# gmarcais/Jellyfish

Hardware: AMD Instinct MI355X
Metric: k-mers/sec at k=21 canonical, 150 bp synthetic reads, bit-exact counts (higher is better)
Workload: dtype u64

## Files before the change

jellyfish_amd/csrc/kernels_p1ring.hip.hpp:

```cpp
#pragma once
#include <type_traits>
#include "kernels_part.hip.hpp"

namespace jfgpu {

template <int P> __device__ __forceinline__ void wave_prio() {
#if defined(__HIP_DEVICE_COMPILE__)
  __builtin_amdgcn_s_setprio(P);
#endif
}

__device__ __forceinline__ uint32_t adm_to_vmask(uint32_t adm) {
  uint32_t r = 0;
#pragma unroll
  for(int j = 0; j < 16; ++j) r |= ((adm >> j) & 1u) << (15 - j);
  return r;
}


constexpr uint32_t kStragPerBlock = 16384;

template <typename ITEM, uint32_t RB = 128> struct Ring {
  static constexpr uint32_t kSlots = RB / sizeof(ITEM);
  static constexpr uint32_t kUnit = 64 / sizeof(ITEM);
// ... 38 lines not shown
  const uint32_t w = s_fill[t];
  uint32_t cnt = w & 0xFFFFu; if(cnt > R::kSlots) cnt = R::kSlots;
  const uint32_t rb = (w >> 16) & (R::kSlots - 1);
  uint32_t units = cnt / R::kUnit; if(all && (cnt % R::kUnit)) ++units;
  uint32_t nout = 0;
  for(uint32_t s = 0; s < units; ++s) {
    uint4 v[4];
    const uint32_t s0 = (rb + s * R::kUnit) & (R::kSlots - 1);
#pragma unroll
    for(int q = 0; q < 4; ++q) v[q] = *reinterpret_cast<const uint4*>(s_ring + t * R::kSlots + ((s0 + R::kChunk * q) & (R::kSlots - 1)));
    if(!all) {
      uint32_t mx = 0;
#pragma unroll
      for(int q = 0; q < 4; ++q) { const uint32_t a = chunk_hole_key<ITEM>(v[q]); mx = mx > a ? mx : a; }
      if(mx == 0xFFFFFFFFu) break;
    }
    if constexpr(!OWNED) {
    if(B.room == 0 && B.nxt_asked) {
      if((uint64_t)B.nxt + kGran <= cap) { B.gpos = B.nxt; B.room = kGran; }
      else { B.exhausted = true; if(B.nxt < cap) atomicMax(&gshort[t], cap - B.nxt); }
      B.nxt_asked = false;
    }
    if(B.room == 0 && !B.exhausted) {
      const uint32_t r0 = atomicAdd(&gcur[t], kGran);
      if((uint64_t)r0 + kGran <= cap) { B.gpos = r0; B.room = kGran; }
      else { B.exhausted = true; if(r0 < cap) atomicMax(&gshort[t], cap - r0); }
    }
    }
    if(B.room) {
      uint4* dst = reinterpret_cast<uint4*>(my_region + B.gpos);
#pragma unroll
      for(int q = 0; q < 4; ++q) dst[q] = v[q];
      const uint32_t real = cnt - s * R::kUnit < R::kUnit ? cnt - s * R::kUnit : R::kUnit;
      B.gpos += OWNED ? real : R::kUnit; B.room -= R::kUnit; B.stored += real;
    } else {
#pragma unroll
      for(int q = 0; q < 4; ++q) chunk_items<ITEM>(v[q], [&](ITEM x) { if(x != hole) straggler(t, x, 1u); });
    }
#pragma unroll
    for(int q = 0; q < 4; ++q)
      *reinterpret_cast<uint4*>(s_ring + t * R::kSlots + ((s0 + R::kChunk * q) & (R::kSlots - 1))) = make_uint4(0xFFFFFFFFu, 0xFFFFFFFFu, 0xFFFFFFFFu, 0xFFFFFFFFu);
    ++nout;
  }
  if constexpr(!OWNED) { if(!all && !B.nxt_asked && !B.exhausted && B.room < R::kSlots) { B.nxt = atomicAdd(&gcur[t], kGran); B.nxt_asked = true; } }
  uint32_t expect = w;
  while(nout || (expect & 0xFFFFu) > R::kSlots) {
    uint32_t c = expect & 0xFFFFu; if(c > R::kSlots) c = R::kSlots;
    const uint32_t taken = nout * R::kUnit < c ? nout * R::kUnit : c;
    const uint32_t neww = ((((expect >> 16) + nout * R::kUnit) & 0xFFFFu) << 16) | (c - taken);
    const uint32_t old = atomicCAS(&s_fill[t], expect, neww);
    if(old == expect) break;
    expect = old;
  }
}

template <typename ITEM, uint32_t RB = 128>
__device__ __forceinline__ void ring_init(ITEM* s_ring, uint32_t* s_fill, uint32_t nb, uint32_t* s_nstrag) {
  using R = Ring<ITEM, RB>;
  for(uint32_t j = threadIdx.x; j < nb; j += blockDim.x) s_fill[j] = R::first_fill(j);
  uint4* r4 = reinterpret_cast<uint4*>(s_ring);
  for(uint32_t j = threadIdx.x; j < nb * (RB / 16) + RB / 16; j += blockDim.x) r4[j] = make_uint4(0xFFFFFFFFu, 0xFFFFFFFFu, 0xFFFFFFFFu, 0xFFFFFFFFu);
  if(threadIdx.x == 0) *s_nstrag = 0;
}

template <typename ITEM>
__device__ __forceinline__ void ring_finish(const RingBooks& B, uint32_t t, ITEM* my_region, uint32_t cap, unsigned int* gshort, unsigned long long* tot) {
  const ITEM hole = (ITEM)~(ITEM)0;
  for(uint32_t r = 0; r < B.room; ++r) my_region[B.gpos + r] = hole;
  if(B.nxt_asked) {
    if((uint64_t)B.nxt + kGran <= cap) { for(uint32_t r = 0; r < kGran; ++r) my_region[B.nxt + r] = hole; }
    else if(B.nxt < cap) atomicMax(&gshort[t], cap - B.nxt);
  }
  if(tot && B.stored) atomicAdd(&tot[t], (unsigned long long)B.stored);
}

struct OneWordDirect {
  static constexpr bool kCountsDirect = true;
  const DevTable* Tm; uint32_t b2; int returning;
  __device__ void operator()(uint32_t b, uint64_t item, uint32_t cnt) const { item_direct_call(Tm, b2, b, item, cnt, returning); }
};
struct RouteListDirect {
  static constexpr bool kCountsDirect = false;
  StragList SL;
  __device__ void operator()(uint32_t b, uint64_t item, uint32_t cnt) const {
    for(uint32_t i = 0; i < cnt; ++i) { const unsigned long long at = atomicAdd(SL.n, 1ull); if(at < SL.cap) SL.rec[at] = ((uint64_t)b << 32) | (uint32_t)item; }
  }
};

template <typename ITEM, bool BLOOM, int NB, int CANON, typename DIRECT = OneWordDirect>
__global__ __launch_bounds__(kPBlock) void p1_ring_kernel(DevTable T, DIRECT D, PartGeom P, const uint8_t* __restrict__ base,
                                                          int64_t lo, int64_t hi, uint32_t cap,
                                                          unsigned int* __restrict__ gcur,
                                                          unsigned long long* __restrict__ tot,
                                                          ITEM* __restrict__ out,
                                                          uint64_t* __restrict__ strag, uint32_t* __restrict__ strag_n) {
  using R = Ring<ITEM>;
  constexpr int RP = sizeof(ITEM) == 4 ? 8 : 4;
  JF_DYN_LDS(s_dyn);
  ITEM* s_ring = reinterpret_cast<ITEM*>(s_dyn);
  __shared__ uint64_t s_fwd[NB < 0 ? 1 : 8 * 256];
  __shared__ uint32_t s_fill[kGranMaxB + 32];
  __shared__ uint32_t s_nstrag;
  __shared__ uint32_t s_codes[kPBlock + 2];
  __shared__ uint32_t s_inv[kPBlock + 2];
  const TableGeom& g = T.g;
  const uint32_t nb = 1u << P.b1;
  const uint32_t t = threadIdx.x, lane = t & 63;
  const bool owner = t < nb;
  const ITEM hole = (ITEM)~(ITEM)0;
  if constexpr(NB >= 0) load_tables_lds(s_fwd, T.fwd_tbl, g.nbytes);
  ring_init<ITEM>(s_ring, s_fill, nb, &s_nstrag);
  const uint32_t dump = nb * R::kSlots + (lane & (R::kSlots - 1));
  [[maybe_unused]] const uint32_t xs_hi_mask = g.lsize_g > 32 ? (g.lsize_g >= 64 ? 0xFFFFFFFFu : ((1u << (g.lsize_g - 32)) - 1u)) : 0u;
  unsigned int* const gshort = gcur + nb;
  uint64_t* const my_strag = strag + (size_t)blockIdx.x * kStragPerBlock * R::kWords;
  const uint32_t k = g.k, bshift = g.lsize_l - P.b1;
  const uint32_t rc_shift = 2 * (k - 1);
  const uint32_t rest_mask = P.rest_shift >= 32 ? 0xFFFFFFFFu : ((1u << P.rest_shift) - 1u);
  RingBooks B;
  if(owner) { B.nxt = atomicAdd(&gcur[t], kGran); B.nxt_asked = true; }
  ITEM* const my_region = out + (uint64_t)t * cap;
  uint32_t my_mers = 0, my_direct = 0;

  auto straggler = [&](uint32_t b, ITEM item, uint32_t cnt) {
    const uint32_t at = atomicAdd(&s_nstrag, 1u);
    if(at < kStragPerBlock) strag_store<ITEM>(my_strag + (size_t)at * R::kWords, b, item, cnt);
    else { D(b, (uint64_t)item, cnt); ++my_direct; }
  };

  const int64_t n_tiles = (hi + kPTilePos - 1) / kPTilePos;
  TileRaw Rw = tile_fetch(base, (int64_t)blockIdx.x * kPTilePos, lo, hi);
  lds_barrier();
  [[maybe_unused]] PhaseClk pc;
  for(int64_t tile = blockIdx.x; tile < n_tiles; tile += gridDim.x) {
    const LaneWords L = tile_stage(Rw, tile * kPTilePos, lo, hi, s_codes, s_inv);
    Rw = tile_fetch(base, (tile + gridDim.x) * kPTilePos, lo, hi);
    JF_PHASE(pc, 0);
    const uint32_t adm = BLOOM ? bloom_admit_mask(T.bloom, g, L) : 0xFFFFu;
    uint64_t fw = (((uint64_t)L.p2 << 32) | L.p1) & g.key_mask;
    uint64_t rc = revcomp64(fw, k);
    uint64_t smear = L.inv48;
    for(uint32_t s = 1; s < k; ) { const uint32_t step = s < k - s ? s : k - s; smear |= smear >> step; s += step; }
    const uint32_t rawmask = ~(uint32_t)smear & 0xFFFFu;
    const uint32_t vmask = BLOOM ? (rawmask & adm_to_vmask(adm)) : rawmask;
    my_mers += (uint32_t)__popc(rawmask);
    auto rounds = [&](auto runs_tag) {
    constexpr bool RUNS = decltype(runs_tag)::value;
    uint64_t pk = 0; uint32_t pv = 0, run = 0;
#pragma unroll 1
    for(int j0 = 0; j0 < kPerLane; j0 += RP) {
      constexpr int NE = RUNS ? RP + 1 : RP;
      uint32_t ea[NE], eo[NE]; ITEM ei[NE];
      [[maybe_unused]] uint32_t spm = 0;
#pragma unroll
      for(int e = 0; e < NE; ++e) { ea[e] = dump; ei[e] = 0; eo[e] = 0; }
      auto emit = [&](int e, uint64_t key, uint32_t cnt, bool on) {
        uint32_t b; ITEM item;
        if constexpr(NB == kHashXS && sizeof(ITEM) == 4) {
          uint32_t ylo, yhi;
          xs_hash_halves<false>((uint32_t)key, (uint32_t)(key >> 32), xs_hi_mask, ylo, yhi);
          b = funnel_r(yhi, ylo, bshift) & (nb - 1);
          item = ((ylo & rest_mask) << g.rem_bits) | ((uint32_t)(key >> 32) >> (g.lsize_g - 32));
        } else {
          const uint64_t pos = NB < 0 ? xs_hash(key, g.lsize_g, g.key_bits) : hash_tables_t<(NB < 0 ? 0 : NB)>(s_fwd, key, g.nbytes);
          b = (uint32_t)(pos >> bshift) & (nb - 1);
          if constexpr(sizeof(ITEM) == 4) item = (((uint32_t)pos & rest_mask) << g.rem_bits) | (uint32_t)(key >> g.lsize_g);
          else item = make_item<ITEM>(g, P, key, pos & g.local_mask);
        }
        const bool special = on && (item == hole || cnt > 1);
        const bool normal = on && !special;
#ifndef JFGPU_P1_LATE_SPECIAL
        if(special) straggler(b, item, cnt);
        const uint32_t o = atomicAdd(&s_fill[normal ? b : nb + (lane & 31u)], 1u);
        ea[e] = normal ? b * R::kSlots : dump; ei[e] = item; eo[e] = normal ? o : 0u;
#else
        const uint32_t o = atomicAdd(&s_fill[normal ? b : nb + (lane & 31u)], 1u);
        spm |= special ? 1u << e : 0u;
        ea[e] = on ? b * R::kSlots : dump; ei[e] = item; eo[e] = normal ? o : special ? (R::kFull | ((cnt < 0xFFFFu ? cnt : 0xFFFFu) << 16)) : 0u;
#endif
      };
#ifndef JFGPU_P1_OLD_EXTRACT
      const uint32_t cur_r = L.cur << (2 * j0), ncur_r = ~cur_r, vm_r = vmask << j0;
#endif
#pragma unroll
      for(int e = 0; e < RP; ++e) {
#ifndef JFGPU_P1_OLD_EXTRACT
        const uint32_t c = (cur_r >> (2 * (15 - e))) & 3u, nc = (ncur_r >> (2 * (15 - e))) & 3u;
        const uint32_t v = vm_r & (1u << (15 - e));
#else
        const int j = j0 + e;
        const uint32_t c = (L.cur >> (2 * (15 - j))) & 3u, nc = 3u - c;
        const uint32_t v = vmask & (1u << (15 - j));
#endif
        if constexpr(NB >= 5 || NB == kHashXS) {
          const uint32_t flo = (uint32_t)fw, fhi = (uint32_t)(fw >> 32), rlo = (uint32_t)rc, rhi = (uint32_t)(rc >> 32);
          fw = ((uint64_t)(funnel_r(fhi, flo, 30) & (uint32_t)(g.key_mask >> 32)) << 32) | ((flo << 2) | c);
          rc = ((uint64_t)((rhi >> 2) | (nc << (rc_shift - 32))) << 32) | funnel_r(rhi, rlo, 2);
        } else {
          fw = ((fw << 2) | c) & g.key_mask;
          rc = (rc >> 2) | ((uint64_t)nc << rc_shift);
        }
        const uint64_t key = ((CANON == 1 || (CANON == 2 && g.canonical)) && rc < fw) ? rc : fw;
        if constexpr(RUNS) {
#ifdef JFGPU_P1_NO_RUNS
          const bool same = false;
#else
          const bool same = v && pv && key == pk;
#endif
          emit(e, pk, run, pv && !same);
          run = same ? run + 1 : 1;
          pk = key; pv = v;
        } else emit(e, key, 1u, v != 0);
      }
      if constexpr(RUNS) { if(j0 + RP >= kPerLane) { emit(NE - 1, pk, run, pv != 0); pv = 0; } }
      uint32_t ghosts = 0;
#pragma unroll
      for(int e = 0; e < NE; ++e) {
        const uint32_t full = eo[e] & R::kFull;
        ghosts |= full;
        const uint32_t at = ea[e] + ((eo[e] + (eo[e] >> 16)) & (R::kSlots - 1));
        s_ring[full ? dump : at] = ei[e];
      }
      if(ghosts) {
#pragma unroll 1
#ifndef JFGPU_P1_LATE_SPECIAL
        for(int e = 0; e < NE; ++e) {
          uint32_t a = 0, o = 0; ITEM it = 0;
#pragma unroll
          for(int q = 0; q < NE; ++q) if(q == e) { a = ea[q]; o = eo[q]; it = ei[q]; }
          if(o & R::kFull) straggler(a / R::kSlots, it, 1u);
        }
#else
        for(int e = 0; e < NE; ++e) if(eo[e] & R::kFull) straggler(ea[e] / R::kSlots, ei[e], ((spm >> e) & 1u) ? eo[e] >> 16 : 1u);
#endif
      }
      JF_PHASE(pc, 1);
      lds_barrier();
      JF_PHASE(pc, 2);
#ifndef JFGPU_P1_NO_FLUSH_PRIO
      wave_prio<3>();
#endif
      if(owner) ring_flush<ITEM>(s_ring, s_fill, t, false, B, my_region, cap, gcur, gshort, straggler);
#ifndef JFGPU_P1_NO_FLUSH_PRIO
      wave_prio<0>();
#endif
      JF_PHASE(pc, 3);
    }
    };
    bool may_run = k < 14;
    {
      const uint32_t hc = L.cur ^ (L.cur >> 2), hp = L.p1 ^ (L.p1 >> 2);
      may_run = may_run || (hc & 0x3FFFu) == 0 || ((hc >> 16) & 0x3FFFu) == 0 || (hp & 0x3FFFu) == 0;
    }
#ifdef JFGPU_P1_ALWAYS_RUNS
    may_run = true;
#endif
    if(__ballot(may_run) != 0ull) rounds(std::true_type{}); else rounds(std::false_type{});
  }
  lds_barrier();
  if(owner) { ring_flush<ITEM>(s_ring, s_fill, t, true, B, my_region, cap, gcur, gshort, straggler); ring_finish<ITEM>(B, t, my_region, cap, gshort, tot); }
  lds_barrier();
  if(t == 0) strag_n[blockIdx.x] = s_nstrag < kStragPerBlock ? s_nstrag : kStragPerBlock;
  JF_PHASE(pc, 4);
  JF_PHASE_FLUSH(pc, 0);
  if(DIRECT::kCountsDirect && my_direct) atomicAdd((unsigned long long*)&T.counters[CTR_DIRECT], (unsigned long long)my_direct);
  uint64_t w = my_mers;
  for(int o = 32; o > 0; o >>= 1) w += __shfl_down(w, o, 64);
  if((threadIdx.x & 63) == 0 && w) atomicAdd((unsigned long long*)&T.counters[CTR_MERS], (unsigned long long)w);
}

template <typename ITEM, typename DIRECT>
__global__ __launch_bounds__(256) void p1_stragglers_kernel(DIRECT D, unsigned long long* __restrict__ ctr_direct, const uint64_t* __restrict__ strag,
                                                            const uint32_t* __restrict__ strag_n, uint32_t n_lists, uint32_t cap,
                                                            unsigned int* __restrict__ gcur, unsigned long long* __restrict__ tot,
                                                            ITEM* __restrict__ out, uint32_t list_cap = kStragPerBlock) {
  using R = Ring<ITEM>;
  uint32_t my_direct = 0;
  for(uint32_t l = blockIdx.x; l < n_lists; l += gridDim.x) {
    const uint32_t n = strag_n[l];
    const uint64_t* rec = strag + (size_t)l * list_cap * R::kWords;
    for(uint32_t i = threadIdx.x; i < n; i += blockDim.x) {
      uint32_t b, cnt; ITEM item;
      strag_load<ITEM>(rec + (size_t)i * R::kWords, b, item, cnt);
      if(cnt == 1 && item != (ITEM)~(ITEM)0) {
        const uint32_t at = atomicAdd(&gcur[b], 1u);
        if(at < cap) { out[(uint64_t)b * cap + at] = item; if(tot) atomicAdd(&tot[b], 1ull); continue; }
        atomicMin(&gcur[b], cap);
// ... 115 lines not shown
        for(int e = 0; e < RP; ++e) it[e] = nx[e];
        r0 += RS;
        load_full(k + 1 < n_full ? r0 : my_a, nx);
        process(it);
      }
    }
    if(r0 < my_b) { uint32_t it[RP]; load_partial(r0, it); process(it); }
  }
  lds_barrier();
  flush(true);
  if(owner) ring_finish<uint32_t>(B, t, my_region, cap, gs, tot ? tot + dest0 : nullptr);
  lds_barrier();
  if(t == 0) strag_n[list] = s_nstrag < kP2StragPerBlock ? s_nstrag : kP2StragPerBlock;
  if(my_direct) atomicAdd(ctr_direct, (unsigned long long)my_direct);
}

template <typename ITEM, int NV, typename DIRECT, int PD = 1>
__global__ __launch_bounds__(kPBlock) void p2_ring_roles_kernel(DIRECT D, uint32_t b2e, uint32_t tag_bits, SegList S, uint32_t cap,
                                                                unsigned int* __restrict__ gcur, ITEM* __restrict__ out, uint32_t bucket0,
                                                                uint64_t* __restrict__ strag, uint32_t* __restrict__ strag_n, unsigned long long* __restrict__ ctr_direct) {
  using R = Ring<ITEM>;
  constexpr int VPI = (int)R::kChunk;
  constexpr int RP = NV * VPI;
  constexpr uint32_t kHalf = kPBlock / 2;
  constexpr uint64_t RS = (uint64_t)kHalf * RP;
  JF_DYN_LDS(s_dyn);
  ITEM* s_ring = reinterpret_cast<ITEM*>(s_dyn);
  __shared__ uint32_t s_fill[kGranMaxB];
  __shared__ uint32_t s_nstrag;
  const uint32_t nb = 1u << b2e;
  const uint32_t bucket = bucket0 + blockIdx.x;
  const uint32_t dest0 = bucket * nb;
  const uint32_t t = threadIdx.x, lane = t & 63;
  const bool storer = t < kHalf;
  const ITEM hole = (ITEM)~(ITEM)0;
  ring_init<ITEM>(s_ring, s_fill, nb, &s_nstrag);
  const uint32_t dump = nb * R::kSlots + (lane & (R::kSlots - 1));
  uint64_t* const my_strag = strag + (size_t)blockIdx.x * kP2StragPerBlock * R::kWords;
  uint32_t my_direct = 0;
  auto straggler = [&](uint32_t d, ITEM item, uint32_t cnt) {
    const uint32_t at = atomicAdd(&s_nstrag, 1u);
    if(at < kP2StragPerBlock) strag_store<ITEM>(my_strag + (size_t)at * R::kWords, dest0 + d, item, cnt);
    else { D(dest0 + d, item, cnt); ++my_direct; }
  };
  lds_barrier();
  auto seg_bounds = [&](uint32_t seg, uint64_t& a, uint64_t& b) { a = seg_lo(S, seg, bucket); b = seg_hi(S, seg, bucket); };
  if(storer) {
    const uint32_t d0 = t, d1 = t + kHalf;
    const bool has0 = d0 < nb, has1 = d1 < nb;
    RingBooks B0, B1;
    B0.room = B1.room = cap & ~(R::kUnit - 1);
    ITEM* const r0p = out + ((uint64_t)dest0 + d0) * cap;
    ITEM* const r1p = out + ((uint64_t)dest0 + d1) * cap;
    auto flush = [&](bool all) {
      if(has0) ring_flush<ITEM, true>(s_ring, s_fill, d0, all, B0, r0p, cap, gcur, gcur, straggler);
      if(has1) ring_flush<ITEM, true>(s_ring, s_fill, d1, all, B1, r1p, cap, gcur, gcur, straggler);
    };
    for(uint32_t seg = 0; seg < S.n; ++seg) {
      uint64_t a, b; seg_bounds(seg, a, b);
      const uint64_t rounds = (b - a + RS - 1) / RS;
#pragma unroll 1
      for(uint64_t r = 0; r < rounds; ++r) { lds_barrier(); flush(false); }
    }
    lds_barrier();
    flush(true);
    if(has0) gcur[dest0 + d0] = B0.gpos;
    if(has1) gcur[dest0 + d1] = B1.gpos;
  } else {
    const uint32_t l = t - kHalf;
    for(uint32_t seg = 0; seg < S.n; ++seg) {
      uint64_t a, b; seg_bounds(seg, a, b);
      const ITEM* src = reinterpret_cast<const ITEM*>(S.items[seg]);
      auto load_full = [&](uint64_t r0, ITEM (&it)[RP]) {
#pragma unroll
        for(int h = 0; h < NV; ++h) {
          const uint4 v = *reinterpret_cast<const uint4*>(src + r0 + (uint64_t)h * kHalf * VPI + (uint64_t)VPI * l);
          int q = 0;
          chunk_items<ITEM>(v, [&](ITEM x) { it[VPI * h + q] = x; ++q; });
        }
      };
      auto load_partial = [&](uint64_t r0, ITEM (&it)[RP]) {
#pragma unroll
        for(int h = 0; h < NV; ++h) {
          const uint64_t i = r0 + (uint64_t)h * kHalf * VPI + (uint64_t)VPI * l;
#pragma unroll
          for(int q = 0; q < VPI; ++q) it[VPI * h + q] = i + q < b ? src[i + q] : hole;
        }
      };
      auto load_exact = [&](uint64_t r0, ITEM (&it)[RP]) {
#pragma unroll 1
        for(int h = 0; h < NV; ++h) {
          const uint64_t i = r0 + (uint64_t)h * kHalf * VPI + (uint64_t)VPI * l;
#pragma unroll
          for(int q = 0; q < VPI; ++q) {
            ITEM x = hole;
            if(i + q < b) { x = src[i + q]; if(x == hole) straggler((uint32_t)(x >> tag_bits) & (nb - 1), x, 1u); }
            it[VPI * h + q] = x;
          }
        }
      };
      auto append = [&](const ITEM (&it)[RP]) {
        uint32_t ea[RP], eo[RP];
#pragma unroll
        for(int e = 0; e < RP; ++e) {
          ea[e] = dump; eo[e] = 0;
          if(it[e] != hole) { const uint32_t d = (uint32_t)(it[e] >> tag_bits) & (nb - 1); ea[e] = d * R::kSlots; eo[e] = atomicAdd(&s_fill[d], 1u); }
        }
        uint32_t ghosts = 0;
#pragma unroll
        for(int e = 0; e < RP; ++e) {
          const uint32_t full = eo[e] & R::kFull;
          ghosts |= full;
          const uint32_t at = ea[e] + ((eo[e] + (eo[e] >> 16)) & (R::kSlots - 1));
          s_ring[full ? dump : at] = it[e];
        }
        if(ghosts) {
#pragma unroll 1
          for(int e = 0; e < RP; ++e) if(eo[e] & R::kFull) straggler(ea[e] / R::kSlots, it[e], 1u);
        }
        lds_barrier();
      };
      uint64_t r0 = a;
      if(S.sh[seg] == 0) {
#pragma unroll 1
        for(; r0 < b; r0 += RS) { ITEM it[RP]; load_exact(r0, it); append(it); }
        continue;
      }
      const uint64_t n_full = (b - a) / RS;
      if(n_full) {
        ITEM nx[PD][RP];
#pragma unroll
        for(int d = 0; d < PD; ++d) load_full((uint64_t)d < n_full ? a + (uint64_t)d * RS : a, nx[d]);
        uint64_t k = 0;
#pragma unroll 1
        for(; k + PD <= n_full; k += PD) {
#pragma unroll
          for(int d = 0; d < PD; ++d) {
            ITEM it[RP];
#pragma unroll
            for(int e = 0; e < RP; ++e) it[e] = nx[d][e];
            const uint64_t nxt = k + d + PD;
            load_full(nxt < n_full ? a + nxt * RS : a, nx[d]);
            append(it);
          }
        }
#pragma unroll
        for(int d = 0; d < PD - 1; ++d)
          if(k + d < n_full) append(nx[d]);
        r0 = a + n_full * RS;
      }
      if(r0 < b) { ITEM it[RP]; load_partial(r0, it); append(it); }
    }
    lds_barrier();
  }
  lds_barrier();
  if(t == 0) strag_n[blockIdx.x] = s_nstrag < kP2StragPerBlock ? s_nstrag : kP2StragPerBlock;
  if(my_direct) atomicAdd(ctr_direct, (unsigned long long)my_direct);
}

}
```

jellyfish_amd/csrc/kmer_core.hpp:

```cpp
#pragma once
#include <stdint.h>

#if defined(__HIPCC__)
#define JF_HD __host__ __device__ __forceinline__
#else
#define JF_HD inline
#endif

namespace jfgpu {

constexpr uint32_t kMaxTileBits = 13;
constexpr uint32_t kMinCountBits = 16;
constexpr uint32_t kMinCountBits32 = 8;

JF_HD uint32_t base_code(uint32_t c) {
  const uint32_t u = c & 0xDFu;
  const uint32_t x = (u >> 1) & 3u;
  const uint32_t code = x ^ (x >> 1);
  const uint32_t valid_set = (1u << 1) | (1u << 3) | (1u << 7) | (1u << 20);
  const bool ok = ((u ^ 0x40u) < 32u) && ((valid_set >> (u & 31u)) & 1u);
  return ok ? code : 4u;
}

JF_HD uint32_t letters_of_codes(uint32_t code) {
// ... 246 lines not shown
JF_HD uint32_t probe_lin(uint32_t idx0, uint32_t p, uint32_t tile_mask) {
  return ((idx0 & ~((1u << kBucketBits) - 1u)) + p) & tile_mask;
}

JF_HD void load16(const uint8_t* p, uint32_t w[4]) {
#if defined(__HIP_DEVICE_COMPILE__)
  const uint4 v = *reinterpret_cast<const uint4*>(p);
  w[0] = v.x; w[1] = v.y; w[2] = v.z; w[3] = v.w;
#else
  for(int i = 0; i < 4; ++i)
    w[i] = (uint32_t)p[4 * i] | ((uint32_t)p[4 * i + 1] << 8) | ((uint32_t)p[4 * i + 2] << 16) | ((uint32_t)p[4 * i + 3] << 24);
#endif
}

constexpr int kPerLane = 16;

JF_HD void load_pack16(const uint8_t* __restrict__ base, int64_t off, int64_t lo, int64_t hi,
                                   uint32_t& codes, uint32_t& inval) {
  if(off + 16 <= lo || off >= hi || off < 0) { codes = 0; inval = 0xFFFFu; return; }
  uint32_t w[4];
  if(off + 16 <= hi) {
    load16(base + off, w);
  } else {
    w[0] = w[1] = w[2] = w[3] = 0;
    for(int i = 0; i < 16 && off + i < hi; ++i) w[i >> 2] |= (uint32_t)base[off + i] << (8 * (i & 3));
  }
  pack16(w, codes, inval);
  if(off < lo) inval |= (0xFFFFu << (16 - (int)(lo - off))) & 0xFFFFu;
  if(off + 16 > hi) inval |= (1u << (int)(off + 16 - hi)) - 1u;
}

struct LaneWords {
  uint32_t cur, p1, p2;
  uint64_t inv48;
};

template <typename F>
JF_HD void for_each_kmer(const TableGeom& g, const LaneWords& L, F&& f) {
  const uint32_t k = g.k;
  uint64_t fw = (((uint64_t)L.p2 << 32) | L.p1) & g.key_mask;
  uint64_t rc = revcomp64(fw, k);
  const uint64_t kwin = k >= 64 ? ~0ull : ((1ull << k) - 1);
  const uint32_t rc_shift = 2 * (k - 1);
#pragma unroll
  for(int j = 0; j < kPerLane; ++j) {
    const uint64_t c = (L.cur >> (2 * (15 - j))) & 3u;
    fw = ((fw << 2) | c) & g.key_mask;
    rc = (rc >> 2) | ((3ull - c) << rc_shift);
    const bool valid = ((L.inv48 >> (15 - j)) & kwin) == 0;
    if(valid) f(j, (g.canonical && rc < fw) ? rc : fw);
  }
}

}
```

jellyfish_amd/csrc/jfgpu.hip:

```cpp
#include <hip/hip_runtime.h>
#include <math.h>
#include <stdint.h>
#include <stdio.h>
#include <string.h>
#include <algorithm>
#include <array>
#include <chrono>
#include <memory>
#include <numeric>
#include <string>
#include <type_traits>
#include <vector>

#include "../../include/jfgpu.h"
#include "gf2_matrix.hpp"
#include "tuning.hpp"
#include "kernels.hip.hpp"
#include "kernels_part.hip.hpp"
#include "kernels_tile.hip.hpp"
#include "kernels_p1ring.hip.hpp"
#include "kernels_bloom.hip.hpp"
#include "kernels_bloom_part.hip.hpp"
#include "kernels_wide.hip.hpp"
#include "kernels_wide_part.hip.hpp"
// ... 676 lines not shown
}

void jfgpu_destroy(jfgpu_table* t) {
  if(!t) return;
  hipSetDevice(t->device);
  if(t->stream) hipStreamSynchronize(t->stream);
  prof_collect(t);
  part_discard(t);
  t->stream2.sync();
  delete t;
}

int jfgpu_get_info(const jfgpu_table* t, jfgpu_info* o) {
  if(!t || !o) return fail(JFGPU_E_INVALID, "null argument");
  memset(o, 0, sizeof(*o));
  o->k = t->g.k; o->key_len = t->g.key_bits; o->canonical = t->g.canonical;
  o->lsize = t->g.lsize_g; o->size = 1ull << t->g.lsize_g; o->local_size = 1ull << t->g.lsize_l;
  o->shard_bits = t->g.shard_bits; o->shard_id = t->g.shard_id;
  o->val_len = t->g.cnt_bits; o->slot_bytes = (uint32_t)slot_bytes_of(t); o->tile_slots = 1u << t->g.tile_bits;
  o->matrix_identity = t->matrix.identity ? 1 : 0;
  o->out_counter_len = t->out_counter_len;
  o->max_reprobe = t->dt.max_probe;
  o->table_bytes = (1ull << t->g.lsize_l) * slot_bytes_of(t);
  return JFGPU_OK;
}

int jfgpu_get_matrix(const jfgpu_table* t, uint64_t* columns) {
  if(!t || !columns) return fail(JFGPU_E_INVALID, "null argument");
  memcpy(columns, t->matrix.columns.data(), sizeof(uint64_t) * t->matrix.c);
  return JFGPU_OK;
}

int jfgpu_clear(jfgpu_table* t) {
  if(t) { t->failed = 0; t->failed_msg.clear(); }
  int rc = use(t); if(rc) return rc;
  part_discard(t);
  HIP_TRY(hipMemsetAsync(t->dt.slots, 0, (1ull << t->g.lsize_l) * slot_bytes_of(t), t->stream));
  HIP_TRY(hipMemsetAsync(t->dt.ovf_key, 0, t->ovf_cap * sizeof(uint64_t), t->stream));
  HIP_TRY(hipMemsetAsync(t->dt.ovf_cnt, 0, t->ovf_cap * sizeof(uint64_t), t->stream));
  HIP_TRY(hipMemsetAsync(t->dt.counters, 0, CTR_COUNT * sizeof(uint64_t), t->stream));
  HIP_TRY(hipMemsetAsync(t->dt.dirty, 0, (size_t)1 << (t->g.lsize_l - t->g.tile_bits), t->stream));
  HIP_TRY(hipStreamSynchronize(t->stream));
  t->pristine = true; t->occ_known = 0; t->fed_since = 0; t->direct_seen = 0; t->occ_bound = 0; t->bigval_bound = 0; t->ovf_failed_need = 0;
  t->flushes_plain = 0; t->flushes_heavy = 0;
  t->n_p2_roles = t->n_p2_ring = t->n_p2_sort = t->n_p2_exact = t->n_p1_ring = t->n_p1_other = t->n_tile_dense = t->n_tile_nword = 0;
  return JFGPU_OK;
}

int jfgpu_sync(jfgpu_table* t) {
  int rc = use(t); if(rc) return rc;
  rc = part_flush(t); if(rc) return rc;
  HIP_TRY(hipStreamSynchronize(t->stream));
#ifdef JFGPU_PHASE_PROF
  { unsigned long long c[24], z[24] = {0};
    if(hipMemcpyFromSymbol(c, HIP_SYMBOL(g_phase_prof), sizeof c) == hipSuccess) {
      fprintf(stderr, "[phase prof] P1 (ring): stage %llu  encode+hash+append %llu  (barrier) %llu  units out %llu  finish %llu\n",
              c[0], c[1], c[2], c[3], c[4]);
      fprintf(stderr, "[phase prof] P2: (barrier) %llu  load %llu  hist %llu  scan %llu  lds-scatter %llu  write-out %llu  finish %llu\n",
              c[8], c[9], c[10], c[11], c[12], c[13], c[14]);
      fprintf(stderr, "[phase prof] T: loop+offsets %llu  rank adds + fill %llu  place %llu  merge %llu  queue (wave 0's own) %llu  (its wait for the others) %llu  store %llu\n",
              c[16], c[17], c[18], c[22], c[21], c[19], c[20]);
      (void)hipMemcpyToSymbol(HIP_SYMBOL(g_phase_prof), z, sizeof z);
    } }
#endif
#ifdef JFGPU_TILE_PROF
  { uint64_t c[CTR_COUNT]; if(read_counters(t, c) == JFGPU_OK)
      fprintf(stderr, "[tile prof] wait+prefetch %llu  fill %llu  insert %llu  store %llu (shader clocks, summed over blocks)\n",
              (unsigned long long)c[CTR_PROF0], (unsigned long long)c[CTR_PROF0 + 1], (unsigned long long)c[CTR_PROF0 + 2], (unsigned long long)c[CTR_PROF0 + 3]); }
#endif
  return check_deferred(t);
}

int jfgpu_wait(jfgpu_table* t) {
  int rc = use(t); if(rc) return rc;
  HIP_TRY(hipStreamSynchronize(t->stream));
  return JFGPU_OK;
}

int jfgpu_count_ascii_dev(jfgpu_table* t, const char* d_bases, size_t n) {
  int rc = use(t); if(rc) return rc;
  if(t->g.shard_bits) return fail(JFGPU_E_INVALID, "sharded table: count through its communicator (jfgpu_comm_count_ascii_dev)");
  if(!d_bases && n) return fail(JFGPU_E_INVALID, "null buffer");
  return launch_count(t, d_bases, n);
}

int jfgpu_count_ascii(jfgpu_table* t, const char* bases, size_t n) {
  int rc = use(t); if(rc) return rc;
  if(t->g.shard_bits) return fail(JFGPU_E_INVALID, "sharded table: count through its communicator (jfgpu_comm_count_ascii_dev)");
  if(!bases && n) return fail(JFGPU_E_INVALID, "null buffer");
  if(n < t->g.k) return JFGPU_OK;
  rc = ensure_stage(t); if(rc) return rc;
  const size_t step = kStageBytes - (t->g.k - 1);
  for(size_t o = 0; o < n; o += step) {
    const size_t len = std::min(kStageBytes, n - o);
    const int b = t->stage_next; t->stage_next ^= 1;
    HIP_TRY(hipEventSynchronize(t->stage_done[b]));
    HIP_TRY(hipMemcpyAsync(t->d_stage[b], bases + o, len, hipMemcpyHostToDevice, t->stream));
    rc = launch_count(t, (const char*)t->d_stage[b].get(), len); if(rc) return rc;
    HIP_TRY(hipEventRecord(t->stage_done[b], t->stream));
    if(o + len >= n) break;
  }
  return JFGPU_OK;
}

static int add_keys_piece(jfgpu_table* t, const uint64_t* d_keys, size_t n, uint64_t val, uint8_t* d_is_new) {
  int rc = JFGPU_OK;
  if(!n) return JFGPU_OK;
  { const bool big = t->g.cnt_bits < 64 && (val >> t->g.cnt_bits) != 0;
    rc = ensure_ovf(t, big ? 0 : (uint64_t)n * val, big ? n : 0); if(rc) return rc; }
  const bool one_word = !t->wide && !t->nword;
  if(one_word && val == 1 && !d_is_new && use_partitioned(t, n * 8)) {
    const int prc = part_ingest(t, (const uint8_t*)d_keys, 0, (int64_t)n, true, n);
    if(prc >= 0) return prc;
  }
// ... 517 lines not shown
```

jellyfish_amd/csrc/kernels.hip.hpp:

```cpp
#pragma once
#include <hip/hip_runtime.h>
#include <stdint.h>
#include "kmer_core.hpp"

namespace jfgpu {

constexpr int kBlock = 256;
constexpr int kPerThread = kPerLane;
constexpr int kTilePos = kBlock * kPerThread;

enum Counter : int { CTR_FULL = 0, CTR_MERS = 1, CTR_OVF_FULL = 2, CTR_OVF_USED = 3, CTR_MISROUTED = 4, CTR_DIRECT = 5,
                     CTR_T_ITEMS = 6, CTR_T_QUEUED = 7 ,
                     CTR_PROF0 = 8 , CTR_COUNT = 12 };

#ifdef JFGPU_PHASE_PROF
__device__ unsigned long long g_phase_prof[24];
struct PhaseClk {
  long long acc[8] = {0, 0, 0, 0, 0, 0, 0, 0}; long long t;
  __device__ PhaseClk() { t = clock64(); }
  __device__ void mark(int i) { const long long n = clock64(); acc[i] += n - t; t = n; }
  __device__ void flush(int base) { if(threadIdx.x == 0) for(int i = 0; i < 8; ++i) if(acc[i]) atomicAdd(&g_phase_prof[base + i], (unsigned long long)acc[i]); }
};
#define JF_PHASE(pc, i) (pc).mark(i)
#define JF_PHASE_FLUSH(pc, base) (pc).flush(base)
#else
struct PhaseClk {};
#define JF_PHASE(pc, i) do {} while(0)
#define JF_PHASE_FLUSH(pc, base) do {} while(0)
#endif

struct DevBloom {
  uint32_t* data;
  uint64_t m;
  uint64_t recip;
  uint32_t nh;
  uint32_t nbytes;
  uint32_t kind;
  uint32_t pad_;
  const uint64_t* tbl1;
  const uint64_t* tbl2;
  uint64_t* cache;
  uint64_t cache_mask;
};

struct DevTable {
  TableGeom g;
  uint64_t* slots;
  const uint64_t* fwd_tbl;
  const uint64_t* inv_tbl;
  uint64_t* ovf_key;
  uint64_t* ovf_cnt;
  uint64_t ovf_mask;
  uint64_t* counters;
  uint32_t max_probe;
  DevBloom bloom;
  uint8_t* dirty;
};

#if defined(JFGPU_EMU)
__device__ __forceinline__ void lds_barrier() { __syncthreads(); }
#define JF_DYN_LDS(name) unsigned char* name = ::hip_emu::dyn_lds()
#else
__device__ __forceinline__ void lds_barrier() { asm volatile("s_waitcnt lgkmcnt(0)\n\ts_barrier" ::: "memory"); }
#define JF_DYN_LDS(name) extern __shared__ __align__(16) unsigned char name[]
#endif

__device__ inline bool bloom_admits(const DevBloom& B, uint64_t key);
__device__ inline uint32_t bloom_admit_mask(const DevBloom& B, const TableGeom& g, const LaneWords& L);

__device__ inline void ovf_add(const DevTable& T, uint64_t slot, uint64_t units) {
  const uint64_t want = slot + 1;
  uint64_t h = (slot * 0x9E3779B97F4A7C15ull) >> 20;
  for(uint64_t p = 0; p <= T.ovf_mask; ++p) {
    const uint64_t s = (h + p) & T.ovf_mask;
    unsigned long long old = atomicCAS((unsigned long long*)&T.ovf_key[s], 0ull, (unsigned long long)want);
    if(old == 0ull) atomicAdd((unsigned long long*)&T.counters[CTR_OVF_USED], 1ull);
    if(old == 0ull || old == want) {
      atomicAdd((unsigned long long*)&T.ovf_cnt[s], (unsigned long long)units);
      return;
    }
  }
// ... 908 lines not shown
```

Before: 15.78 billion.

## Extract k-mers by direct funnel shifts and use mask-select bitops in emit

```diff
diff --git a/jellyfish_amd/csrc/kernels_p1ring.hip.hpp b/jellyfish_amd/csrc/kernels_p1ring.hip.hpp
--- a/jellyfish_amd/csrc/kernels_p1ring.hip.hpp
+++ b/jellyfish_amd/csrc/kernels_p1ring.hip.hpp
@@ -177,7 +177,11 @@
   unsigned int* const gshort = gcur + nb;
   uint64_t* const my_strag = strag + (size_t)blockIdx.x * kStragPerBlock * R::kWords;
   const uint32_t k = g.k, bshift = g.lsize_l - P.b1;
-  const uint32_t rc_shift = 2 * (k - 1);
+  constexpr bool EXTRACT = NB >= 5 || NB == kHashXS;
+  constexpr bool MASKS = EXTRACT;
+  [[maybe_unused]] const uint32_t bo_mask = (nb - 1) << 2;
+  [[maybe_unused]] const uint32_t spare_bo = (nb + (lane & 31u)) << 2;
+  [[maybe_unused]] const uint32_t rc_shift = 2 * (k - 1), hi_bits = 2 * k - 32;
   const uint32_t rest_mask = P.rest_shift >= 32 ? 0xFFFFFFFFu : ((1u << P.rest_shift) - 1u);
   RingBooks B;
   if(owner) { B.nxt = atomicAdd(&gcur[t], kGran); B.nxt_asked = true; }
@@ -199,8 +203,10 @@
     Rw = tile_fetch(base, (tile + gridDim.x) * kPTilePos, lo, hi);
     JF_PHASE(pc, 0);
     const uint32_t adm = BLOOM ? bloom_admit_mask(T.bloom, g, L) : 0xFFFFu;
-    uint64_t fw = (((uint64_t)L.p2 << 32) | L.p1) & g.key_mask;
-    uint64_t rc = revcomp64(fw, k);
+    [[maybe_unused]] uint64_t fw = 0, rc = 0;
+    [[maybe_unused]] RcString V{};
+    if constexpr(EXTRACT) V = rc_string(L, k);
+    else { fw = (((uint64_t)L.p2 << 32) | L.p1) & g.key_mask; rc = revcomp64(fw, k); }
     uint64_t smear = L.inv48;
     for(uint32_t s = 1; s < k; ) { const uint32_t step = s < k - s ? s : k - s; smear |= smear >> step; s += step; }
     const uint32_t rawmask = ~(uint32_t)smear & 0xFFFFu;
@@ -212,53 +218,43 @@
 #pragma unroll 1
     for(int j0 = 0; j0 < kPerLane; j0 += RP) {
       constexpr int NE = RUNS ? RP + 1 : RP;
-      uint32_t ea[NE], eo[NE]; ITEM ei[NE];
-      [[maybe_unused]] uint32_t spm = 0;
-#pragma unroll
-      for(int e = 0; e < NE; ++e) { ea[e] = dump; ei[e] = 0; eo[e] = 0; }
-      auto emit = [&](int e, uint64_t key, uint32_t cnt, bool on) {
+      uint32_t ea[NE], eo[NE]; [[maybe_unused]] uint32_t em[NE]; ITEM ei[NE];
+#pragma unroll
+      for(int e = 0; e < NE; ++e) { ea[e] = MASKS ? 0u : dump; ei[e] = 0; eo[e] = 0; em[e] = 0; }
+      auto emit = [&](int e, uint64_t key, uint32_t cnt, uint32_t m) {
         uint32_t b; ITEM item;
         if constexpr(NB == kHashXS && sizeof(ITEM) == 4) {
           uint32_t ylo, yhi;
           xs_hash_halves<false>((uint32_t)key, (uint32_t)(key >> 32), xs_hi_mask, ylo, yhi);
-          b = funnel_r(yhi, ylo, bshift) & (nb - 1);
+          b = funnel_r(yhi, ylo, bshift - 2) & bo_mask;
           item = ((ylo & rest_mask) << g.rem_bits) | ((uint32_t)(key >> 32) >> (g.lsize_g - 32));
         } else {
           const uint64_t pos = NB < 0 ? xs_hash(key, g.lsize_g, g.key_bits) : hash_tables_t<(NB < 0 ? 0 : NB)>(s_fwd, key, g.nbytes);
-          b = (uint32_t)(pos >> bshift) & (nb - 1);
+          b = ((uint32_t)(pos >> bshift) & (nb - 1)) << (MASKS ? 2 : 0);
           if constexpr(sizeof(ITEM) == 4) item = (((uint32_t)pos & rest_mask) << g.rem_bits) | (uint32_t)(key >> g.lsize_g);
           else item = make_item<ITEM>(g, P, key, pos & g.local_mask);
         }
-        const bool special = on && (item == hole || cnt > 1);
-        const bool normal = on && !special;
-#ifndef JFGPU_P1_LATE_SPECIAL
-        if(special) straggler(b, item, cnt);
-        const uint32_t o = atomicAdd(&s_fill[normal ? b : nb + (lane & 31u)], 1u);
-        ea[e] = normal ? b * R::kSlots : dump; ei[e] = item; eo[e] = normal ? o : 0u;
-#else
-        const uint32_t o = atomicAdd(&s_fill[normal ? b : nb + (lane & 31u)], 1u);
-        spm |= special ? 1u << e : 0u;
-        ea[e] = on ? b * R::kSlots : dump; ei[e] = item; eo[e] = normal ? o : special ? (R::kFull | ((cnt < 0xFFFFu ? cnt : 0xFFFFu) << 16)) : 0u;
-#endif
+        if constexpr(MASKS) {
+          if(item == hole || cnt > 1) { if(m) straggler(b >> 2, item, cnt); m = 0; }
+          eo[e] = atomicAdd(reinterpret_cast<uint32_t*>(reinterpret_cast<unsigned char*>(s_fill) + mask_select(b, spare_bo, m)), 1u);
+          ea[e] = b; ei[e] = item; em[e] = m;
+        } else {
+          const bool special = m && (item == hole || cnt > 1);
+          const bool normal = m && !special;
+          if(special) straggler(b, item, cnt);
+          const uint32_t o = atomicAdd(&s_fill[normal ? b : nb + (lane & 31u)], 1u);
+          ea[e] = normal ? b * R::kSlots : dump; ei[e] = item; eo[e] = normal ? o : 0u;
+        }
       };
-#ifndef JFGPU_P1_OLD_EXTRACT
-      const uint32_t cur_r = L.cur << (2 * j0), ncur_r = ~cur_r, vm_r = vmask << j0;
-#endif
+      const uint32_t vm_r = vmask << j0;
+      [[maybe_unused]] const uint32_t cur_r = L.cur << (2 * j0), ncur_r = ~cur_r;
+      [[maybe_unused]] const RoundStrings<RP, sizeof(ITEM) == 4> W(L, V, j0);
 #pragma unroll
       for(int e = 0; e < RP; ++e) {
-#ifndef JFGPU_P1_OLD_EXTRACT
-        const uint32_t c = (cur_r >> (2 * (15 - e))) & 3u, nc = (ncur_r >> (2 * (15 - e))) & 3u;
-        const uint32_t v = vm_r & (1u << (15 - e));
-#else
-        const int j = j0 + e;
-        const uint32_t c = (L.cur >> (2 * (15 - j))) & 3u, nc = 3u - c;
-        const uint32_t v = vmask & (1u << (15 - j));
-#endif
-        if constexpr(NB >= 5 || NB == kHashXS) {
-          const uint32_t flo = (uint32_t)fw, fhi = (uint32_t)(fw >> 32), rlo = (uint32_t)rc, rhi = (uint32_t)(rc >> 32);
-          fw = ((uint64_t)(funnel_r(fhi, flo, 30) & (uint32_t)(g.key_mask >> 32)) << 32) | ((flo << 2) | c);
-          rc = ((uint64_t)((rhi >> 2) | (nc << (rc_shift - 32))) << 32) | funnel_r(rhi, rlo, 2);
-        } else {
+        const uint32_t v = MASKS ? bit_mask(vm_r, 15 - e) : vm_r & (1u << (15 - e));
+        if constexpr(EXTRACT) W.mers(e, hi_bits, (uint32_t)(g.key_mask >> 32), fw, rc);
+        else {
+          const uint32_t c = (cur_r >> (2 * (15 - e))) & 3u, nc = (ncur_r >> (2 * (15 - e))) & 3u;
           fw = ((fw << 2) | c) & g.key_mask;
           rc = (rc >> 2) | ((uint64_t)nc << rc_shift);
         }
@@ -269,32 +265,36 @@
 #else
           const bool same = v && pv && key == pk;
 #endif
-          emit(e, pk, run, pv && !same);
+          emit(e, pk, run, same ? 0u : pv);
           run = same ? run + 1 : 1;
           pk = key; pv = v;
-        } else emit(e, key, 1u, v != 0);
+        } else emit(e, key, 1u, v);
       }
-      if constexpr(RUNS) { if(j0 + RP >= kPerLane) { emit(NE - 1, pk, run, pv != 0); pv = 0; } }
+      if constexpr(RUNS) { if(j0 + RP >= kPerLane) { emit(NE - 1, pk, run, pv); pv = 0; } }
       uint32_t ghosts = 0;
 #pragma unroll
       for(int e = 0; e < NE; ++e) {
-        const uint32_t full = eo[e] & R::kFull;
-        ghosts |= full;
-        const uint32_t at = ea[e] + ((eo[e] + (eo[e] >> 16)) & (R::kSlots - 1));
-        s_ring[full ? dump : at] = ei[e];
+        if constexpr(MASKS) {
+          const uint32_t away = full_or_none(eo[e], R::kFull, em[e]);
+          ghosts = or_and(ghosts, eo[e], em[e]);
+          const uint32_t at = (ea[e] << 3) + ((eo[e] + (eo[e] >> 16)) & (R::kSlots - 1));
+          s_ring[away ? dump : at] = ei[e];
+        } else {
+          const uint32_t full = eo[e] & R::kFull;
+          ghosts |= full;
+          const uint32_t at = ea[e] + ((eo[e] + (eo[e] >> 16)) & (R::kSlots - 1));
+          s_ring[full ? dump : at] = ei[e];
+        }
       }
+      ghosts &= R::kFull;
       if(ghosts) {
 #pragma unroll 1
-#ifndef JFGPU_P1_LATE_SPECIAL
         for(int e = 0; e < NE; ++e) {
           uint32_t a = 0, o = 0; ITEM it = 0;
 #pragma unroll
-          for(int q = 0; q < NE; ++q) if(q == e) { a = ea[q]; o = eo[q]; it = ei[q]; }
-          if(o & R::kFull) straggler(a / R::kSlots, it, 1u);
-        }
-#else
-        for(int e = 0; e < NE; ++e) if(eo[e] & R::kFull) straggler(ea[e] / R::kSlots, ei[e], ((spm >> e) & 1u) ? eo[e] >> 16 : 1u);
-#endif
+          for(int q = 0; q < NE; ++q) if(q == e) { a = ea[q]; o = MASKS ? eo[q] & em[q] : eo[q]; it = ei[q]; }
+          if(o & R::kFull) straggler(MASKS ? a >> 2 : a / R::kSlots, it, 1u);
+        }
       }
       JF_PHASE(pc, 1);
       lds_barrier();
diff --git a/jellyfish_amd/csrc/kmer_core.hpp b/jellyfish_amd/csrc/kmer_core.hpp
--- a/jellyfish_amd/csrc/kmer_core.hpp
+++ b/jellyfish_amd/csrc/kmer_core.hpp
@@ -322,4 +322,72 @@
   }
 }
 
-}
+JF_HD uint32_t bfe_u32(uint32_t x, uint32_t off, uint32_t width) {
+#if defined(__HIP_DEVICE_COMPILE__)
+  return __builtin_amdgcn_ubfe(x, off, width);
+#else
+  return (x >> off) & ((1u << width) - 1u);
+#endif
+}
+JF_HD uint32_t bit_mask(uint32_t x, uint32_t bit) {
+#if defined(__HIP_DEVICE_COMPILE__)
+  return (uint32_t)__builtin_amdgcn_sbfe((int32_t)x, bit, 1);
+#else
+  return 0u - ((x >> bit) & 1u);
+#endif
+}
+JF_HD uint32_t mask_select(uint32_t a, uint32_t b, uint32_t m) {
+#if defined(__HIP_DEVICE_COMPILE__)
+  return __builtin_amdgcn_bitop3_b32(a, b, m, 0xE4);
+#else
+  return (a & m) | (b & ~m);
+#endif
+}
+JF_HD uint32_t or_and(uint32_t a, uint32_t b, uint32_t c) {
+#if defined(__HIP_DEVICE_COMPILE__)
+  return __builtin_amdgcn_bitop3_b32(a, b, c, 0xF8);
+#else
+  return a | (b & c);
+#endif
+}
+JF_HD uint32_t full_or_none(uint32_t o, uint32_t full, uint32_t m) {
+#if defined(__HIP_DEVICE_COMPILE__)
+  return __builtin_amdgcn_bitop3_b32(o, full, m, 0xD5);
+#else
+  return (o & full) | ~m;
+#endif
+}
+JF_HD uint32_t revcomp32(uint32_t x) {
+  x = ~x;
+#if defined(__HIP_DEVICE_COMPILE__)
+  x = __builtin_bitreverse32(x);
+  return ((x >> 1) & 0x55555555u) | ((x & 0x55555555u) << 1);
+#else
+  x = ((x >> 2) & 0x33333333u) | ((x & 0x33333333u) << 2);
+  x = ((x >> 4) & 0x0F0F0F0Fu) | ((x & 0x0F0F0F0Fu) << 4);
+  x = ((x >> 8) & 0x00FF00FFu) | ((x & 0x00FF00FFu) << 8);
+  return (x >> 16) | (x << 16);
+#endif
+}
+struct RcString { uint32_t v0, v1, v2; };
+JF_HD RcString rc_string(const LaneWords& L, uint32_t k) {
+  const uint32_t t0 = revcomp32(L.p2), t1 = revcomp32(L.p1), t2 = revcomp32(L.cur), s = 2 * (32 - k);
+  return RcString{funnel_r(t1, t0, s), funnel_r(t2, t1, s), t2 >> s};
+}
+template <int RP, bool NARROW> struct RoundStrings {
+  uint32_t a0, a1, a2, u0, u1, u2;
+  JF_HD RoundStrings(const LaneWords& L, const RcString& V, int j0) {
+    const uint32_t sf = 2 * (kPerLane - RP - j0), sr = 2 * j0;
+    a0 = funnel_r(L.p1, L.cur, sf); a1 = funnel_r(L.p2, L.p1, sf); a2 = NARROW ? 0u : L.p2 >> sf;
+    u0 = funnel_r(V.v1, V.v0, sr); u1 = funnel_r(V.v2, V.v1, sr); u2 = NARROW ? 0u : V.v2 >> sr;
+  }
+  JF_HD void mers(int e, uint32_t hi_bits, uint32_t hi_mask, uint64_t& fw, uint64_t& rc) const {
+    const uint32_t f = 2 * (RP - 1 - e), r = 2 * (1 + e);
+    const uint32_t flo = funnel_r(a1, a0, f), rlo = funnel_r(u1, u0, r);
+    const uint32_t fhi = NARROW ? bfe_u32(a1, f, hi_bits) : funnel_r(a2, a1, f) & hi_mask;
+    const uint32_t rhi = NARROW ? bfe_u32(u1, r, hi_bits) : funnel_r(u2, u1, r) & hi_mask;
+    fw = ((uint64_t)fhi << 32) | flo; rc = ((uint64_t)rhi << 32) | rlo;
+  }
+};
+
+}
```

Measured after the change: 15.90 billion, median of 2. About the same (+0.8%).

## Fuse the two owned-ring flushes in P2 roles and batch the release CAS

Applied to the files above, without the earlier changes.

```diff
diff --git a/jellyfish_amd/csrc/jfgpu.hip b/jellyfish_amd/csrc/jfgpu.hip
--- a/jellyfish_amd/csrc/jfgpu.hip
+++ b/jellyfish_amd/csrc/jfgpu.hip
@@ -752,7 +752,7 @@
   rc = part_flush(t); if(rc) return rc;
   HIP_TRY(hipStreamSynchronize(t->stream));
 #ifdef JFGPU_PHASE_PROF
-  { unsigned long long c[24], z[24] = {0};
+  { unsigned long long c[40], z[40] = {0};
     if(hipMemcpyFromSymbol(c, HIP_SYMBOL(g_phase_prof), sizeof c) == hipSuccess) {
       fprintf(stderr, "[phase prof] P1 (ring): stage %llu  encode+hash+append %llu  (barrier) %llu  units out %llu  finish %llu\n",
               c[0], c[1], c[2], c[3], c[4]);
@@ -760,6 +760,10 @@
               c[8], c[9], c[10], c[11], c[12], c[13], c[14]);
       fprintf(stderr, "[phase prof] T: loop+offsets %llu  rank adds + fill %llu  place %llu  merge %llu  queue (wave 0's own) %llu  (its wait for the others) %llu  store %llu\n",
               c[16], c[17], c[18], c[22], c[21], c[19], c[20]);
+      fprintf(stderr, "[phase prof] P2 roles, storer wave 0: (barrier) %llu  fill read %llu  chunk reads + test %llu  stores + resets %llu  release %llu  rest %llu"
+                      "  | lanes releasing %llu  failed compare-and-swaps %llu\n", c[24], c[25], c[26], c[27], c[28], c[29], c[30], c[31]);
+      fprintf(stderr, "[phase prof] P2 roles, loader wave 8: wait for items %llu  rank adds %llu  ring stores %llu  (barrier) %llu  rest %llu\n",
+              c[32], c[33], c[34], c[35], c[37]);
       (void)hipMemcpyToSymbol(HIP_SYMBOL(g_phase_prof), z, sizeof z);
     } }
 #endif
diff --git a/jellyfish_amd/csrc/kernels.hip.hpp b/jellyfish_amd/csrc/kernels.hip.hpp
--- a/jellyfish_amd/csrc/kernels.hip.hpp
+++ b/jellyfish_amd/csrc/kernels.hip.hpp
@@ -14,19 +14,31 @@
                      CTR_PROF0 = 8 , CTR_COUNT = 12 };
 
 #ifdef JFGPU_PHASE_PROF
-__device__ unsigned long long g_phase_prof[24];
+__device__ unsigned long long g_phase_prof[40];
 struct PhaseClk {
   long long acc[8] = {0, 0, 0, 0, 0, 0, 0, 0}; long long t;
+  unsigned cnt[2] = {0, 0};
   __device__ PhaseClk() { t = clock64(); }
   __device__ void mark(int i) { const long long n = clock64(); acc[i] += n - t; t = n; }
-  __device__ void flush(int base) { if(threadIdx.x == 0) for(int i = 0; i < 8; ++i) if(acc[i]) atomicAdd(&g_phase_prof[base + i], (unsigned long long)acc[i]); }
+  __device__ void flush(int base, unsigned tid = 0) { if(threadIdx.x == tid) for(int i = 0; i < 8; ++i) if(acc[i]) atomicAdd(&g_phase_prof[base + i], (unsigned long long)acc[i]); }
+  __device__ void flush_counts(int base, unsigned tid) { if(threadIdx.x - tid < 64u) for(int i = 0; i < 2; ++i) if(cnt[i]) atomicAdd(&g_phase_prof[base + i], (unsigned long long)cnt[i]); }
 };
 #define JF_PHASE(pc, i) (pc).mark(i)
 #define JF_PHASE_FLUSH(pc, base) (pc).flush(base)
+#define JF_PHASE_FLUSH_AS(pc, base, tid) (pc).flush(base, tid)
+#define JF_PHASE_LDS_BACK() asm volatile("s_waitcnt lgkmcnt(0)" ::: "memory")
+#define JF_PHASE_TOUCH(x) asm volatile("" :: "v"(x) : "memory")
+#define JF_PHASE_COUNT(pc, i, n) ((pc).cnt[i] += (n))
+#define JF_PHASE_FLUSH_COUNTS(pc, base, tid) (pc).flush_counts(base, tid)
 #else
 struct PhaseClk {};
 #define JF_PHASE(pc, i) do {} while(0)
 #define JF_PHASE_FLUSH(pc, base) do {} while(0)
+#define JF_PHASE_FLUSH_AS(pc, base, tid) do {} while(0)
+#define JF_PHASE_LDS_BACK() do {} while(0)
+#define JF_PHASE_TOUCH(x) do {} while(0)
+#define JF_PHASE_COUNT(pc, i, n) do {} while(0)
+#define JF_PHASE_FLUSH_COUNTS(pc, base, tid) do {} while(0)
 #endif
 
 struct DevBloom {
diff --git a/jellyfish_amd/csrc/kernels_p1ring.hip.hpp b/jellyfish_amd/csrc/kernels_p1ring.hip.hpp
--- a/jellyfish_amd/csrc/kernels_p1ring.hip.hpp
+++ b/jellyfish_amd/csrc/kernels_p1ring.hip.hpp
@@ -114,6 +114,100 @@
     if(old == expect) break;
     expect = old;
   }
+}
+
+template <typename R> __device__ __forceinline__ uint32_t ring_released(uint32_t expect, uint32_t nout) {
+  uint32_t c = expect & 0xFFFFu; if(c > R::kSlots) c = R::kSlots;
+  const uint32_t taken = nout * R::kUnit < c ? nout * R::kUnit : c;
+  return ((((expect >> 16) + nout * R::kUnit) & 0xFFFFu) << 16) | (c - taken);
+}
+
+template <typename ITEM, typename STRAG>
+__device__ __forceinline__ void ring_flush_owned2(ITEM* s_ring, uint32_t* s_fill, uint32_t d0, uint32_t d1, bool has0, bool has1, RingBooks& B0, RingBooks& B1,
+                                                  ITEM* region0, ITEM* region1, PhaseClk& pc, STRAG&& straggler) {
+  using R = Ring<ITEM>;
+  const ITEM hole = (ITEM)~(ITEM)0;
+  const uint4 holes4 = make_uint4(0xFFFFFFFFu, 0xFFFFFFFFu, 0xFFFFFFFFu, 0xFFFFFFFFu);
+  ITEM* const ring0 = s_ring + d0 * R::kSlots;
+  ITEM* const ring1 = s_ring + d1 * R::kSlots;
+  uint32_t w0 = 0, w1 = 0;
+  if(has0) w0 = s_fill[d0];
+  if(has1) w1 = s_fill[d1];
+  JF_PHASE_LDS_BACK(); JF_PHASE(pc, 1);
+  const uint32_t c0 = (w0 & 0xFFFFu) < R::kSlots ? (w0 & 0xFFFFu) : R::kSlots, c1 = (w1 & 0xFFFFu) < R::kSlots ? (w1 & 0xFFFFu) : R::kSlots;
+  const uint32_t p0 = (w0 >> 16) & (R::kSlots - 1), p1 = (w1 >> 16) & (R::kSlots - 1);
+  uint4 a[4] = {holes4, holes4, holes4, holes4}, b[4] = {holes4, holes4, holes4, holes4};
+  if(c0 >= R::kUnit) {
+#pragma unroll
+    for(int q = 0; q < 4; ++q) a[q] = *reinterpret_cast<const uint4*>(ring0 + ((p0 + R::kChunk * q) & (R::kSlots - 1)));
+  }
+  if(c1 >= R::kUnit) {
+#pragma unroll
+    for(int q = 0; q < 4; ++q) b[q] = *reinterpret_cast<const uint4*>(ring1 + ((p1 + R::kChunk * q) & (R::kSlots - 1)));
+  }
+  auto complete = [&](const uint4 (&v)[4]) {
+    uint32_t mx = 0;
+#pragma unroll
+    for(int q = 0; q < 4; ++q) { const uint32_t k = chunk_hole_key<ITEM>(v[q]); mx = mx > k ? mx : k; }
+    return mx != 0xFFFFFFFFu;
+  };
+  const bool out0 = complete(a), out1 = complete(b);
+  JF_PHASE_LDS_BACK(); JF_PHASE(pc, 2);
+  constexpr uint32_t kNoRoom = 0xFFFFFFFFu;
+  auto take = [&](RingBooks& B) {
+    if(!B.room) return kNoRoom;
+    const uint32_t at = B.gpos;
+    B.gpos += R::kUnit; B.room -= R::kUnit; B.stored += R::kUnit;
+    return at;
+  };
+  auto reset = [&](ITEM* ring, uint32_t s0) {
+#pragma unroll
+    for(int q = 0; q < 4; ++q) *reinterpret_cast<uint4*>(ring + ((s0 + R::kChunk * q) & (R::kSlots - 1))) = holes4;
+  };
+  auto put = [&](const uint4 (&v)[4], uint32_t at, uint32_t d, ITEM* region) {
+    if(at != kNoRoom) {
+      uint4* dst = reinterpret_cast<uint4*>(region + at);
+#pragma unroll
+      for(int q = 0; q < 4; ++q) dst[q] = v[q];
+    } else {
+#pragma unroll
+      for(int q = 0; q < 4; ++q) chunk_items<ITEM>(v[q], [&](ITEM x) { if(x != hole) straggler(d, x, 1u); });
+    }
+  };
+  uint32_t n0 = 0, n1 = 0, at0 = kNoRoom, at1 = kNoRoom;
+  if(out0) { at0 = take(B0); reset(ring0, p0); n0 = 1; }
+  if(out1) { at1 = take(B1); reset(ring1, p1); n1 = 1; }
+  auto second = [&](ITEM* ring, uint32_t p, uint32_t d, RingBooks& B, ITEM* region) {
+    uint4 v[4];
+    const uint32_t s0 = (p + R::kUnit) & (R::kSlots - 1);
+#pragma unroll
+    for(int q = 0; q < 4; ++q) v[q] = *reinterpret_cast<const uint4*>(ring + ((s0 + R::kChunk * q) & (R::kSlots - 1)));
+    if(!complete(v)) return 0u;
+    put(v, take(B), d, region);
+    reset(ring, s0);
+    return 1u;
+  };
+  if(out0 && c0 == R::kSlots) n0 += second(ring0, p0, d0, B0, region0);
+  if(out1 && c1 == R::kSlots) n1 += second(ring1, p1, d1, B1, region1);
+  bool rel0 = n0 || (w0 & 0xFFFFu) > R::kSlots, rel1 = n1 || (w1 & 0xFFFFu) > R::kSlots;
+  uint32_t e0 = w0, e1 = w1, o0 = w0, o1 = w1;
+  JF_PHASE_COUNT(pc, 0, (uint32_t)rel0 + (uint32_t)rel1);
+  if(rel0) o0 = atomicCAS(&s_fill[d0], e0, ring_released<R>(e0, n0));
+  if(rel1) o1 = atomicCAS(&s_fill[d1], e1, ring_released<R>(e1, n1));
+  if(out0) put(a, at0, d0, region0);
+  if(out1) put(b, at1, d1, region1);
+  JF_PHASE(pc, 3);
+  rel0 = o0 != e0; rel1 = o1 != e1;
+  e0 = o0; e1 = o1;
+  JF_PHASE_COUNT(pc, 1, (uint32_t)rel0 + (uint32_t)rel1);
+  while(rel0 || rel1) {
+    if(rel0) o0 = atomicCAS(&s_fill[d0], e0, ring_released<R>(e0, n0));
+    if(rel1) o1 = atomicCAS(&s_fill[d1], e1, ring_released<R>(e1, n1));
+    rel0 = o0 != e0; rel1 = o1 != e1;
+    e0 = o0; e1 = o1;
+    JF_PHASE_COUNT(pc, 1, (uint32_t)rel0 + (uint32_t)rel1);
+  }
+  JF_PHASE_LDS_BACK(); JF_PHASE(pc, 4);
 }
 
 template <typename ITEM, uint32_t RB = 128>
@@ -516,21 +610,29 @@
     B0.room = B1.room = cap & ~(R::kUnit - 1);
     ITEM* const r0p = out + ((uint64_t)dest0 + d0) * cap;
     ITEM* const r1p = out + ((uint64_t)dest0 + d1) * cap;
-    auto flush = [&](bool all) {
-      if(has0) ring_flush<ITEM, true>(s_ring, s_fill, d0, all, B0, r0p, cap, gcur, gcur, straggler);
-      if(has1) ring_flush<ITEM, true>(s_ring, s_fill, d1, all, B1, r1p, cap, gcur, gcur, straggler);
-    };
+    PhaseClk pc;
     for(uint32_t seg = 0; seg < S.n; ++seg) {
       uint64_t a, b; seg_bounds(seg, a, b);
       const uint64_t rounds = (b - a + RS - 1) / RS;
-#pragma unroll 1
-      for(uint64_t r = 0; r < rounds; ++r) { lds_barrier(); flush(false); }
+      JF_PHASE(pc, 5);
+#pragma unroll 1
+      for(uint64_t r = 0; r < rounds; ++r) {
+        lds_barrier();
+        JF_PHASE(pc, 0);
+        ring_flush_owned2<ITEM>(s_ring, s_fill, d0, d1, has0, has1, B0, B1, r0p, r1p, pc, straggler);
+      }
     }
     lds_barrier();
-    flush(true);
+    JF_PHASE(pc, 0);
+    if(has0) ring_flush<ITEM, true>(s_ring, s_fill, d0, true, B0, r0p, cap, gcur, gcur, straggler);
+    if(has1) ring_flush<ITEM, true>(s_ring, s_fill, d1, true, B1, r1p, cap, gcur, gcur, straggler);
     if(has0) gcur[dest0 + d0] = B0.gpos;
     if(has1) gcur[dest0 + d1] = B1.gpos;
+    JF_PHASE(pc, 5);
+    JF_PHASE_FLUSH(pc, 24);
+    JF_PHASE_FLUSH_COUNTS(pc, 30, 0);
   } else {
+    [[maybe_unused]] PhaseClk pc;
     const uint32_t l = t - kHalf;
     for(uint32_t seg = 0; seg < S.n; ++seg) {
       uint64_t a, b; seg_bounds(seg, a, b);
@@ -565,11 +667,16 @@
       };
       auto append = [&](const ITEM (&it)[RP]) {
         uint32_t ea[RP], eo[RP];
+        JF_PHASE(pc, 5);
+#pragma unroll
+        for(int e = 0; e < RP; ++e) JF_PHASE_TOUCH(it[e]);
+        JF_PHASE(pc, 0);
 #pragma unroll
         for(int e = 0; e < RP; ++e) {
           ea[e] = dump; eo[e] = 0;
           if(it[e] != hole) { const uint32_t d = (uint32_t)(it[e] >> tag_bits) & (nb - 1); ea[e] = d * R::kSlots; eo[e] = atomicAdd(&s_fill[d], 1u); }
         }
+        JF_PHASE_LDS_BACK(); JF_PHASE(pc, 1);
         uint32_t ghosts = 0;
 #pragma unroll
         for(int e = 0; e < RP; ++e) {
@@ -582,7 +689,9 @@
 #pragma unroll 1
           for(int e = 0; e < RP; ++e) if(eo[e] & R::kFull) straggler(ea[e] / R::kSlots, it[e], 1u);
         }
+        JF_PHASE_LDS_BACK(); JF_PHASE(pc, 2);
         lds_barrier();
+        JF_PHASE(pc, 3);
       };
       uint64_t r0 = a;
       if(S.sh[seg] == 0) {
@@ -616,6 +725,8 @@
       if(r0 < b) { ITEM it[RP]; load_partial(r0, it); append(it); }
     }
     lds_barrier();
+    JF_PHASE(pc, 5);
+    JF_PHASE_FLUSH_AS(pc, 32, kHalf);
   }
   lds_barrier();
   if(t == 0) strag_n[blockIdx.x] = s_nstrag < kP2StragPerBlock ? s_nstrag : kP2StragPerBlock;
```

After: 15.70 billion before, 15.92 billion after, median of 3. No clear change (+1.3%).
